# mttga/purejaxql

Hardware: NVIDIA H100
Metric: MinAtar-Breakout env steps/sec @4096 envs x128 seeds (higher is better)
Workload: dtype f32

## Files before the change

include/pqn_b200.h:

```cpp
#ifndef PQN_B200_H
#define PQN_B200_H

#include <stdint.h>

#ifdef __cplusplus
extern "C" {
#endif

#define PQN_OK 0
#define PQN_E_INVALID (-1)
#define PQN_E_CUDA (-2)
#define PQN_E_UNSUPPORTED (-3)

#define PQN_ENV_BREAKOUT 0
#define PQN_ENV_ASTERIX 1
#define PQN_ENV_SPACE_INVADERS 2
#define PQN_ENV_FREEWAY 3
#define PQN_ENV_SEAQUEST 4
#define PQN_ENV_CARTPOLE 16
#define PQN_ENV_ACROBOT 17
#define PQN_ENV_MEMORY_CHAIN 32

typedef struct pqn_env_info_t {
  int32_t state_words;
// ... 103 lines not shown
                 int32_t E, void* workspace, void* stream);
int pqn_rnn_loss_grad(const pqn_net_desc_t* desc_host, const float* params, const float* hs0, const float* obs,
                      const uint8_t* last_done, const int32_t* last_action, const int32_t* action, const float* reward,
                      const uint8_t* done, float* grads, float* loss_sum, float* qsa_sum, int32_t S, int32_t T, int32_t B,
                      float gamma, float lambda, void* workspace, void* stream);

int pqn_radam_clip_step(float* params, const float* grads, float* mu, float* nu, const float* sched,
                        int32_t* step_counter, float* gnorm_scratch , int32_t S, int64_t P,
                        float max_norm, float b1, float b2, float eps, void* stream);

int pqn_bn_stats_update(float* batch_stats, float* bn_sums, int32_t S, int32_t F, int64_t stats_seed_stride,
                        float count, float momentum, void* stream);

int pqn_set_tensor_core_path(int on);
int pqn_set_conv_mma_path(int on);

int pqn_tc_split_lo(const float* x, float* lo, int64_t n, void* stream);
int pqn_tc_gemm_test(const float* a, const float* a_lo, const float* b, const float* b_lo, float* d, int32_t S,
                     int32_t M, int32_t N, int32_t K, int a_mn, int b_mn, int split3, void* stream);

int pqn_tc_split16(const float* x, void* hi, void* lo, int64_t n, float scale, void* stream);
int pqn_tc_gemm16_test(const void* a_hi, const void* a_lo, const void* b_hi, const void* b_lo, float* d, int32_t S,
                       int32_t M, int32_t N, int32_t K, int a_mn, int b_mn, float out_scale, void* stream);
int pqn_tc_dgrad16_test(const void* a_hi, const void* a_lo, const void* b_hi, const void* b_lo, const float* mask,
                        const uint32_t* relu_bits, float* d, int32_t S, int32_t M, int32_t N, int32_t K, int epi,
                        float out_scale, void* stream);

#ifdef __cplusplus
}
#endif
// ... 2 lines not shown
```

purejaxql_b200/_lib.py:

```python
from __future__ import annotations

import ctypes
import os
from ctypes import POINTER, Structure, c_char_p, c_double, c_float, c_int, c_int32, c_int64, c_longlong, c_void_p

HERE = os.path.dirname(os.path.abspath(__file__))
LIB_PATH = os.path.join(HERE, "libpqn_b200.so")


class EnvInfo(Structure):
    _fields_ = [("state_words", c_int32), ("obs_dim", c_int32), ("obs_shape", c_int32 * 3),
                ("num_actions", c_int32), ("max_steps", c_int32), ("binary_obs", c_int32),
                ("packed_obs_words", c_int32)]


class EnvParams(Structure):
    _fields_ = [("max_steps", c_int32), ("memory_length", c_int32)]


class NetDesc(Structure):
    _fields_ = [("kind", c_int32), ("in_c", c_int32), ("hidden", c_int32), ("layers", c_int32),
                ("num_actions", c_int32), ("norm_type", c_int32), ("norm_input", c_int32)]


# ... 47 lines not shown
    "pqn_qnet_forward": (c_int, [POINTER(NetDesc), c_void_p, c_void_p, c_void_p, c_void_p, c_int64, c_void_p, c_int32,
                                 c_int64, c_void_p, c_void_p]),
    "pqn_qnet_loss_grad": (c_int, [POINTER(NetDesc), c_void_p, c_void_p, c_void_p, c_void_p, c_int64, c_void_p,
                                   c_void_p, c_int64, c_void_p, c_void_p, c_void_p, c_void_p, c_int32, c_int64,
                                   c_void_p, c_void_p]),
    "pqn_rnn_step": (c_int, [POINTER(NetDesc), c_void_p, c_void_p, c_void_p, c_int64, c_void_p, c_void_p, c_void_p,
                             c_int32, c_int32, c_void_p, c_void_p]),
    "pqn_rnn_loss_grad": (c_int, [POINTER(NetDesc), c_void_p, c_void_p, c_void_p, c_void_p, c_void_p, c_void_p, c_void_p,
                                  c_void_p, c_void_p, c_void_p, c_void_p, c_int32, c_int32, c_int32, c_float, c_float,
                                  c_void_p, c_void_p]),
    "pqn_radam_clip_step": (c_int, [c_void_p, c_void_p, c_void_p, c_void_p, c_void_p, c_void_p, c_void_p, c_int32,
                                    c_int64, c_float, c_float, c_float, c_float, c_void_p]),
    "pqn_bn_stats_update": (c_int, [c_void_p, c_void_p, c_int32, c_int32, c_int64, c_float, c_float, c_void_p]),
    "pqn_set_tensor_core_path": (c_int, [c_int]),
    "pqn_set_conv_mma_path": (c_int, [c_int]),
    "pqn_tc_split_lo": (c_int, [c_void_p, c_void_p, c_int64, c_void_p]),
    "pqn_tc_split16": (c_int, [c_void_p, c_void_p, c_void_p, c_int64, c_float, c_void_p]),
    "pqn_tc_gemm_test": (c_int, [c_void_p, c_void_p, c_void_p, c_void_p, c_void_p, c_int32, c_int32, c_int32,
                                 c_int32, c_int, c_int, c_int, c_void_p]),
    "pqn_tc_gemm16_test": (c_int, [c_void_p, c_void_p, c_void_p, c_void_p, c_void_p, c_int32, c_int32, c_int32,
                                   c_int32, c_int, c_int, c_float, c_void_p]),
    "pqn_tc_dgrad16_test": (c_int, [c_void_p, c_void_p, c_void_p, c_void_p, c_void_p, c_void_p, c_void_p, c_int32,
                                    c_int32, c_int32, c_int32, c_int, c_float, c_void_p]),
}

EXPORTS = tuple(_SIGS)
_lib = None


def lib():
# ... 52 lines not shown
```

purejaxql_b200/csrc/pqn_net.cu:

```cuda
#include <cuda_runtime.h>
#include <stdint.h>

#include "../../include/pqn_b200.h"
#include "api_common.h"
#include "tc_common.cuh"

namespace pqn {

constexpr int GT = 256;
constexpr int BK = 16;
constexpr float LN_EPS = 1e-6f;
constexpr int CONV_O = 16;
constexpr int CONV_PIX = 64;
constexpr int HID_CNN = 128;
constexpr int FLAT_CNN = CONV_PIX * CONV_O;

static int g_use_tc = 2;
static int g_conv_mma = 1;

static inline int64_t align4(int64_t x) { return (x + 3) & ~(int64_t)3; }

static int make_layout(const pqn_net_desc_t* d, pqn_net_layout_t* L) {
  int64_t off = 0;
  auto take = [&](int64_t n) { int64_t o = off; off += align4(n); return o; };
// ... 1003 lines not shown
    for (int h = 0; h < 2; ++h) {
      bl[h] = wb_lo[(ks * 2 + h) * 32 + lane];
      bh[h] = wb_hi[(ks * 2 + h) * 32 + lane];
    }
#pragma unroll
    for (int h = 0; h < 2; ++h)
#pragma unroll
      for (int i = 0; i < 2; ++i) mma_tf32_16n8k8(z[i][h], a[i], __float_as_uint(bl[h].x), __float_as_uint(bl[h].y));
#pragma unroll
    for (int h = 0; h < 2; ++h)
#pragma unroll
      for (int i = 0; i < 2; ++i) mma_tf32_16n8k8(z[i][h], a[i], __float_as_uint(bh[h].x), __float_as_uint(bh[h].y));
  }
}

__device__ __forceinline__ void ln16_quad(const float (&z)[2][4], float& mean0, float& rstd0, float& mean1,
                                          float& rstd1) {
  float s0 = z[0][0] + z[0][1] + z[1][0] + z[1][1];
  float q0 = z[0][0] * z[0][0] + z[0][1] * z[0][1] + z[1][0] * z[1][0] + z[1][1] * z[1][1];
  float s1 = z[0][2] + z[0][3] + z[1][2] + z[1][3];
  float q1 = z[0][2] * z[0][2] + z[0][3] * z[0][3] + z[1][2] * z[1][2] + z[1][3] * z[1][3];
#pragma unroll
  for (int o = 1; o <= 2; o <<= 1) {
    s0 += __shfl_xor_sync(0xffffffffu, s0, o); q0 += __shfl_xor_sync(0xffffffffu, q0, o);
    s1 += __shfl_xor_sync(0xffffffffu, s1, o); q1 += __shfl_xor_sync(0xffffffffu, q1, o);
  }
  mean0 = s0 * (1.0f / CONV_O); mean1 = s1 * (1.0f / CONV_O);
  rstd0 = rsqrtf(fmaxf(q0 * (1.0f / CONV_O) - mean0 * mean0, 0.f) + LN_EPS);
  rstd1 = rsqrtf(fmaxf(q1 * (1.0f / CONV_O) - mean1 * mean1, 0.f) + LN_EPS);
}

constexpr int CONV_MMA_WARPS = 8;

template <int C, bool TRAIN, bool H16 = false>
__global__ void __launch_bounds__(CONV_MMA_WARPS * 32, 3)
    conv_fwd_mma_kernel(const uint32_t* __restrict__ obs, int64_t obs_rows_per_seed, const int32_t* __restrict__ gather,
                        const float* __restrict__ params, int64_t P, pqn_net_layout_t L, float* __restrict__ H1,
                        float* __restrict__ H1LO, float* __restrict__ XH1, float* __restrict__ RS1,
                        uint32_t* __restrict__ RB, float* __restrict__ bn_sums, int rows) {
  using Cfg = ConvCfg<C>;
  using M = ConvMma<C>;
  __shared__ float2 wb_hi[M::KS * 2 * 32], wb_lo[M::KS * 2 * 32];
  __shared__ float cb[CONV_O], sc[CONV_O], bi[CONV_O];
  __shared__ uint32_t so[CONV_MMA_WARPS][Cfg::SW];
// ... 120 lines not shown
  }
}

__device__ __forceinline__ void mma_f16_16n8k16(float (&d)[4], const uint32_t (&a)[4], uint32_t b0, uint32_t b1) {
  asm volatile(
      "mma.sync.aligned.m16n8k16.row.col.f32.f16.f16.f32 {%0,%1,%2,%3}, {%4,%5,%6,%7}, {%8,%9}, {%0,%1,%2,%3};"
      : "+f"(d[0]), "+f"(d[1]), "+f"(d[2]), "+f"(d[3])
      : "r"(a[0]), "r"(a[1]), "r"(a[2]), "r"(a[3]), "r"(b0), "r"(b1));
}

template <int C>
struct Conv16 {
  static constexpr int TAPS = 9 * C;
  static constexpr int KS = (TAPS + 15) / 16;
  static constexpr int ROW = 2 * KS < 8 ? 8 : 2 * KS;
};

__host__ __device__ constexpr int conv16_channel(int h, int n) { return 4 * (n >> 1) + 2 * h + (n & 1); }

__host__ __device__ constexpr int conv16_tap(int s, int kk) {
  return 16 * s + (kk < 8 ? 0 : 8) + ((kk & 1) ? 4 : 0) + ((kk & 7) >> 1);
}

template <int C>
__device__ __forceinline__ void conv16_load_weights(const float* __restrict__ prm, const pqn_net_layout_t& L, uint4* wb,
                                                    float* cb, float* sc, float* bi) {
  using M = Conv16<C>;
  const float inv255 = 1.0f / 255.0f;
  for (int i = threadIdx.x; i < M::KS * 2 * 32; i += blockDim.x) {
    const int ln = i & 31, h = (i >> 5) & 1, s = i >> 6;
    const int gg = ln >> 2, tt = ln & 3;
    const int o = conv16_channel(h, gg);
    const float scale = __uint_as_float((uint32_t)(127 + 15 - (1 << tt)) << 23);
    float v[4];
#pragma unroll
    for (int q = 0; q < 4; ++q) {
      const int tap = conv16_tap(s, 2 * tt + (q & 1) + (q >> 1) * 8);
      v[q] = tap < M::TAPS ? __ldg(prm + L.conv_w + tap * CONV_O + o) * inv255 * scale : 0.f;
      v[q] = fminf(fmaxf(v[q], -65000.f), 65000.f);
    }
    const __half2 h0 = __floats2half2_rn(v[0], v[1]), h1 = __floats2half2_rn(v[2], v[3]);
    const float2 f0 = __half22float2(h0), f1 = __half22float2(h1);
    const __half2 l0 = __floats2half2_rn(v[0] - f0.x, v[1] - f0.y), l1 = __floats2half2_rn(v[2] - f1.x, v[3] - f1.y);
    wb[i] = make_uint4(*reinterpret_cast<const uint32_t*>(&h0), *reinterpret_cast<const uint32_t*>(&h1),
                       *reinterpret_cast<const uint32_t*>(&l0), *reinterpret_cast<const uint32_t*>(&l1));
  }
  if (threadIdx.x < CONV_O) {
    cb[threadIdx.x] = __ldg(prm + L.conv_b + threadIdx.x);
    sc[threadIdx.x] = __ldg(prm + L.ln0_scale + threadIdx.x);
    bi[threadIdx.x] = __ldg(prm + L.ln0_bias + threadIdx.x);
  }
}

template <int C>
__device__ __forceinline__ void build_patch16(const uint32_t* __restrict__ so, int pix, uint32_t* __restrict__ out) {
  constexpr int W = PatchCfg<C>::WORDS;
  uint32_t w[W];
  patch_bits<C>(so, pix, w);
#pragma unroll
  for (int b = 0; b < 2 * Conv16<C>::KS; ++b) {
    const int o = 8 * b;
    uint32_t v = (o >> 5) < W ? w[(o >> 5) < W ? (o >> 5) : 0] : 0u;
    const int sh = o & 31;
    const uint32_t lo = sh >= 10 ? v >> (sh - 10) : v << (10 - sh);
    const uint32_t hi = sh + 4 <= 26 ? v << (26 - sh - 4) : v >> (sh + 4 - 26);
// ... 26 lines not shown
      z[i][h][0] = z[i][h][2] = cb[4 * t + 2 * h];
      z[i][h][1] = z[i][h][3] = cb[4 * t + 2 * h + 1];
    }
  const uint32_t* r00 = xp + (32 * mbp + g) * M::ROW;
#pragma unroll
  for (int s = 0; s < M::KS; ++s) {
    uint32_t a[2][4];
#pragma unroll
    for (int i = 0; i < 2; ++i) {
      const uint2 w0 = *reinterpret_cast<const uint2*>(r00 + (16 * i) * M::ROW + 2 * s);
      const uint2 w1 = *reinterpret_cast<const uint2*>(r00 + (16 * i + 8) * M::ROW + 2 * s);
      a[i][0] = w0.x & mask; a[i][1] = w1.x & mask; a[i][2] = w0.y & mask; a[i][3] = w1.y & mask;
    }
    uint4 b[2];
#pragma unroll
    for (int h = 0; h < 2; ++h) b[h] = wb[(s * 2 + h) * 32 + lane];
#pragma unroll
    for (int h = 0; h < 2; ++h)
#pragma unroll
      for (int i = 0; i < 2; ++i) mma_f16_16n8k16(z[i][h], a[i], b[h].z, b[h].w);
#pragma unroll
    for (int h = 0; h < 2; ++h)
#pragma unroll
      for (int i = 0; i < 2; ++i) mma_f16_16n8k16(z[i][h], a[i], b[h].x, b[h].y);
  }
}

__device__ __forceinline__ uint32_t cvt_f16x2_satfinite(float lo, float hi) {
  uint32_t r;
  asm("cvt.rn.satfinite.f16x2.f32 %0, %1, %2;" : "=r"(r) : "f"(hi), "f"(lo));
  return r;
}

constexpr int CONV16_WARPS = 4;
constexpr int CONV16_CTAS_PER_SM = 5;

template <int C, bool TRAIN, bool H16>
__global__ void __launch_bounds__(CONV16_WARPS * 32, CONV16_CTAS_PER_SM)
    conv_fwd_mma16_kernel(const uint32_t* __restrict__ obs, int64_t obs_rows_per_seed, const int32_t* __restrict__ gather,
                          const float* __restrict__ params, int64_t P, pqn_net_layout_t L, float* __restrict__ H1,
                          float* __restrict__ H1LO, float* __restrict__ XH1, float* __restrict__ RS1,
                          uint32_t* __restrict__ RB, float* __restrict__ bn_sums, int rows) {
  using Cfg = ConvCfg<C>;
  using M = Conv16<C>;
  __shared__ __align__(16) uint4 wb[M::KS * 2 * 32];
  __shared__ float cb[CONV_O], sc[CONV_O], bi[CONV_O];
  __shared__ uint32_t so[CONV16_WARPS][Cfg::SW];
  __shared__ __align__(16) uint32_t sxp[CONV16_WARPS][CONV_PIX * M::ROW];
  __shared__ float s_cnt[C];
  const int tid = threadIdx.x, warp = tid >> 5, lane = tid & 31;
  const int g = lane >> 2, t = lane & 3;
  const int seed = blockIdx.y;
  conv16_load_weights<C>(params + (int64_t)seed * P, L, wb, cb, sc, bi);
  if (TRAIN && tid < C) s_cnt[tid] = 0.f;
  __syncthreads();
  int cnt[C];
  uint32_t cmask[C];
#pragma unroll
  for (int c = 0; c < C; ++c) {
    cnt[c] = 0;
// ... 31 lines not shown
    src_next = fetch_index(row + 2 * row_stride);
    store_patch16<C>(my_so, lane, sxp[warp] + lane * M::ROW);
    store_patch16<C>(my_so, lane + 32, sxp[warp] + (lane + 32) * M::ROW);
    __syncwarp();
    const int64_t grow = (int64_t)seed * rows + row;
    float* __restrict__ hrow = H16 ? nullptr : H1 + grow * FLAT_CNN;
    __half* __restrict__ hrow16 = H16 ? reinterpret_cast<__half*>(H1) + grow * FLAT_CNN : nullptr;
    __half* __restrict__ lrow16 = H16 ? reinterpret_cast<__half*>(H1LO) + grow * FLAT_CNN : nullptr;
    float* __restrict__ xrow = (TRAIN && XH1) ? XH1 + grow * FLAT_CNN : nullptr;
    float* __restrict__ rrow = (TRAIN && RS1) ? RS1 + grow * CONV_PIX : nullptr;
    uint16_t* __restrict__ brow = (TRAIN && RB) ? reinterpret_cast<uint16_t*>(RB + grow * (FLAT_CNN / 32)) : nullptr;
    float keep_rs0 = 0.f, keep_rs1 = 0.f;
    uint32_t keep_rb = 0u;
#pragma unroll 1
    for (int mbp = 0; mbp < 2; ++mbp) {
      float z2[2][2][4];
      conv16_block2<C>(sxp[warp], wb, cb, mbp, lane, z2);
#pragma unroll
      for (int mi = 0; mi < 2; ++mi) {
        const int mb = 2 * mbp + mi;
        float (&z)[2][4] = z2[mi];
        float mean0, rstd0, mean1, rstd1;
        ln16_quad(z, mean0, rstd0, mean1, rstd1);
        const float nm0 = -mean0 * rstd0, nm1 = -mean1 * rstd1;
        uint32_t rb0 = 0u, rb1 = 0u;
        const int p0 = 16 * mb + g, p1 = p0 + 8, o4 = 4 * t;
        float x0[4], x1[4], v0[4], v1[4];
#pragma unroll
        for (int h = 0; h < 2; ++h) {
#pragma unroll
          for (int c = 0; c < 2; ++c) {
            const int o = o4 + 2 * h + c;
            x0[2 * h + c] = fmaf(z[h][c], rstd0, nm0);
            x1[2 * h + c] = fmaf(z[h][2 + c], rstd1, nm1);
            v0[2 * h + c] = fmaxf(fmaf(x0[2 * h + c], sc[o], bi[o]), 0.f);
            v1[2 * h + c] = fmaxf(fmaf(x1[2 * h + c], sc[o], bi[o]), 0.f);
          }
        }
        if (H16) {
          uint32_t hw0[2], hw1[2], lw0[2], lw1[2];
#pragma unroll
          for (int h = 0; h < 2; ++h) {
            hw0[h] = cvt_f16x2_satfinite(v0[2 * h], v0[2 * h + 1]);
            hw1[h] = cvt_f16x2_satfinite(v1[2 * h], v1[2 * h + 1]);
            const float2 f0 = __half22float2(*reinterpret_cast<const __half2*>(&hw0[h]));
            const float2 f1 = __half22float2(*reinterpret_cast<const __half2*>(&hw1[h]));
            const __half2 l0 = __floats2half2_rn((v0[2 * h] - f0.x) * tc::TC_LO_SCALE, (v0[2 * h + 1] - f0.y) * tc::TC_LO_SCALE);
            const __half2 l1 = __floats2half2_rn((v1[2 * h] - f1.x) * tc::TC_LO_SCALE, (v1[2 * h + 1] - f1.y) * tc::TC_LO_SCALE);
            lw0[h] = *reinterpret_cast<const uint32_t*>(&l0); lw1[h] = *reinterpret_cast<const uint32_t*>(&l1);
          }
          *reinterpret_cast<uint2*>(hrow16 + p0 * CONV_O + o4) = make_uint2(hw0[0], hw0[1]);
          *reinterpret_cast<uint2*>(lrow16 + p0 * CONV_O + o4) = make_uint2(lw0[0], lw0[1]);
// ... 274 lines not shown
  }
  float* __restrict__ o = part + ((int64_t)seed * gridDim.x + blockIdx.x) * (M::TAPS * CONV_O + 3 * CONV_O);
  for (int i = tid; i < M::TAPS * CONV_O; i += blockDim.x) o[i] = s_w[i] * (1.0f / 255.0f);
  if (tid < 3 * CONV_O) o[M::TAPS * CONV_O + tid] = s_red[tid];
}

template <int C>
struct ConvBwd16 {
  static constexpr int MT = ConvMma<C>::MT;
  static constexpr int NG = 4 * MT;
  static constexpr int NGP = (NG % 8 == 4) ? NG : NG + 4;
  static constexpr int DY = 0;
  static constexpr int XH = DY + FLAT_CNN;
  static constexpr int RS = XH + FLAT_CNN;
  static constexpr int DZT = RS + CONV_PIX;
  static constexpr int PW = DZT + 2 * CONV_O * 32;
  static constexpr int WARP_FLOATS = (PW + 32 * NGP + 3) / 4 * 4;
  static constexpr int WARPS = (C == 4) ? 8 : 6;
  static constexpr int BYTES = (WARPS * WARP_FLOATS + 4 * CONV_O) * 4;
};

__device__ __forceinline__ int cswz16(int p, int col) {
  return ((p ^ ((p >> 2) & 1)) << 4) + (col ^ (((p >> 1) & 1) << 3));
}
__device__ __forceinline__ int dzt_word(int ch, int ks, int pos) {
  const int c7 = ch & 7;
  return (ch << 5) + ((ks ^ ((c7 + (c7 >> 2)) & 3)) << 3) + pos;
}

template <int C>
__global__ void __launch_bounds__(ConvBwd16<C>::WARPS * 32, 2)
    conv_bwd_mma16_kernel(const uint32_t* __restrict__ obs, int64_t obs_rows_per_seed, const int32_t* __restrict__ gather,
                          const float* __restrict__ params, int64_t P, pqn_net_layout_t L, const float* __restrict__ DY1,
                          const float* __restrict__ XH1, const float* __restrict__ RS1, float* __restrict__ part,
                          int rows, float gs) {
  using Cfg = ConvCfg<C>;
  using M = ConvMma<C>;
  using SM = ConvBwd16<C>;
  constexpr int PWD = PatchCfg<C>::WORDS;
  extern __shared__ __align__(16) float smem_bwd[];
  const int tid = threadIdx.x, warp = tid >> 5, lane = tid & 31;
  const int g = lane >> 2, t = lane & 3;
  const int seed = blockIdx.y;
  float* my = smem_bwd + warp * SM::WARP_FLOATS;
  float* my_dy = my + SM::DY;
  float* my_xh = my + SM::XH;
  float* my_rs = my + SM::RS;
  uint32_t* my_dzt = reinterpret_cast<uint32_t*>(my + SM::DZT);
  uint32_t* my_so = reinterpret_cast<uint32_t*>(my + SM::DZT);
  uint32_t* my_pw = reinterpret_cast<uint32_t*>(my + SM::PW);
  float* sc = smem_bwd + SM::WARPS * SM::WARP_FLOATS;
  float* s_red = sc + CONV_O;
  float* s_w = smem_bwd;
  static_assert(Cfg::SW <= 2 * CONV_O * 32, "obs staging aliases the dz planes");
  static_assert(M::MT * 16 * CONV_O <= SM::WARP_FLOATS * SM::WARPS, "dW reduction buffer aliases the warp slices");
  static_assert(Cfg::PW <= 32, "one packed observation word per lane");
  if (tid < CONV_O) sc[tid] = __ldg(params + (int64_t)seed * P + L.ln0_scale + tid);
  if (tid < 3 * CONV_O) s_red[tid] = 0.f;
  __syncthreads();
  float a_dsc[4] = {0.f, 0.f, 0.f, 0.f}, a_dbi[4] = {0.f, 0.f, 0.f, 0.f}, a_dcb[4] = {0.f, 0.f, 0.f, 0.f};
  float wrun[M::MT][2][4];
#pragma unroll
  for (int mt = 0; mt < M::MT; ++mt)
#pragma unroll
    for (int h = 0; h < 2; ++h)
#pragma unroll
      for (int j = 0; j < 4; ++j) wrun[mt][h][j] = 0.f;
  const uint32_t amask = (1u << (10 + (g & 3))) | (1u << (26 + (g & 3)));
  const int pos_g = g < 4 ? 2 * g : 2 * (g - 4) + 1;

  const int row_stride = gridDim.x * SM::WARPS;
  auto fetch_index = [&](int r) -> int {
    const int rc = r < rows ? r : rows - 1;
    return gather ? __ldg(gather + (int64_t)seed * rows + rc) : rc;
  };
  auto fetch_obs = [&](int src) -> uint32_t {
    return __ldg(obs + ((int64_t)seed * obs_rows_per_seed + src) * Cfg::PW + (lane < Cfg::PW ? lane : 0));
  };
  auto fetch_rows = [&](int r) {
    if (r < rows) {
      const int64_t gr = (int64_t)seed * rows + r;
      const float* dsrc = DY1 + gr * FLAT_CNN;
      const float* xsrc = XH1 + gr * FLAT_CNN;
#pragma unroll
      for (int i = 0; i < FLAT_CNN / 4 / 32; ++i) {
        const int q = i * 32 + lane, prow = q >> 2;
        const int dst = cswz16(prow, (q & 3) * 4);
        cp_async16(my_dy + dst, dsrc + q * 4);
        cp_async16(my_xh + dst, xsrc + q * 4);
      }
      if (lane < CONV_PIX / 4) cp_async16(my_rs + lane * 4, RS1 + gr * CONV_PIX + lane * 4);
    }
    cp_async_commit();
  };
  int row = blockIdx.x * SM::WARPS + warp;
  uint32_t pre = fetch_obs(fetch_index(row));
  int src_next = fetch_index(row + row_stride);
  fetch_rows(row);
  for (; row < rows; row += row_stride) {
    __syncwarp();
    if (lane < Cfg::PW) my_so[lane] = pre;
    if (lane == 0) my_so[Cfg::PW] = 0u;
    __syncwarp();
    pre = fetch_obs(src_next);
    src_next = fetch_index(row + 2 * row_stride);
    {
      uint32_t w0[PWD], w1[PWD];
      patch_bits<C>(my_so, 2 * lane, w0);
      patch_bits<C>(my_so, 2 * lane + 1, w1);
      uint32_t pw[SM::NGP];
#pragma unroll
      for (int k = 0; k < SM::NGP; ++k) pw[k] = 0u;
#pragma unroll
      for (int q = 0; q < SM::NG; ++q) {
        const int ql = q & 3, slot = (q & ~3) + (ql == 1 ? 2 : (ql == 2 ? 1 : ql));
        const int bit = 4 * q, wi = bit >> 5, sh = bit & 31;
        if (wi < PWD) {
          const uint32_t v0 = w0[wi < PWD ? wi : 0], v1 = w1[wi < PWD ? wi : 0];
          const uint32_t lo = sh >= 10 ? v0 >> (sh >= 10 ? sh - 10 : 0) : v0 << (sh < 10 ? 10 - sh : 0);
          const uint32_t hi = sh <= 26 ? v1 << (sh <= 26 ? 26 - sh : 0) : v1 >> (sh > 26 ? sh - 26 : 0);
          pw[slot] = __byte_perm(lo, hi, 0x7610);
        }
      }
      uint32_t* dstw = my_pw + lane * SM::NGP;
#pragma unroll
      for (int k = 0; k < SM::NGP / 4; ++k)
        *reinterpret_cast<uint4*>(dstw + 4 * k) = make_uint4(pw[4 * k], pw[4 * k + 1], pw[4 * k + 2], pw[4 * k + 3]);
    }
    cp_async_wait_all();
    __syncwarp();
#pragma unroll 1
    for (int mb = 0; mb < 4; ++mb) {
      const int p0 = 16 * mb + 2 * g, p1 = p0 + 1;
      float z[2][4];
      float2 dyv[2][2];
#pragma unroll
      for (int h = 0; h < 2; ++h) {
        dyv[h][0] = *reinterpret_cast<const float2*>(my_dy + cswz16(p0, 8 * h + 2 * t));
        dyv[h][1] = *reinterpret_cast<const float2*>(my_dy + cswz16(p1, 8 * h + 2 * t));
        const float2 a0 = *reinterpret_cast<const float2*>(my_xh + cswz16(p0, 8 * h + 2 * t));
        const float2 a1 = *reinterpret_cast<const float2*>(my_xh + cswz16(p1, 8 * h + 2 * t));
        z[h][0] = a0.x; z[h][1] = a0.y; z[h][2] = a1.x; z[h][3] = a1.y;
      }
// ... 68 lines not shown
        a[0] = wa.x & amask; a[1] = wa.y & amask; a[2] = wb.x & amask; a[3] = wb.y & amask;
        mma_f16_16n8k16(wacc[mt][0], a, blo[0].x, blo[0].y);
        mma_f16_16n8k16(wacc[mt][1], a, blo[1].x, blo[1].y);
        mma_f16_16n8k16(wacc[mt][0], a, bhi[0].x, bhi[0].y);
        mma_f16_16n8k16(wacc[mt][1], a, bhi[1].x, bhi[1].y);
      }
    }
#pragma unroll
    for (int mt = 0; mt < M::MT; ++mt)
#pragma unroll
      for (int h = 0; h < 2; ++h)
#pragma unroll
        for (int j = 0; j < 4; ++j) wrun[mt][h][j] += wacc[mt][h][j];
  }
  cp_async_wait_all();
  const float inv_gs = 1.0f / gs;
  const float unscale = __uint_as_float((uint32_t)(127 + 15 - (1 << (g & 3))) << 23) * inv_gs;
  __syncthreads();
  for (int w = 0; w < SM::WARPS; ++w) {
    if (warp == w) {
#pragma unroll
      for (int mt = 0; mt < M::MT; ++mt)
#pragma unroll
        for (int h = 0; h < 2; ++h)
#pragma unroll
          for (int j = 0; j < 4; ++j) {
            const int tap = 16 * mt + g + (j >= 2 ? 8 : 0);
            float* dst = &s_w[tap * CONV_O + 8 * h + 2 * t + (j & 1)];
            *dst = (w == 0 ? 0.f : *dst) + wrun[mt][h][j] * unscale;
          }
// ... 247 lines not shown
  if (cudaFuncSetAttribute(kfn, cudaFuncAttributeMaxDynamicSharedMemorySize, ConvBwdSmem<C>::BYTES) != cudaSuccess)
    return check_launch("conv_bwd_mma(cudaFuncSetAttribute)");
  kfn<<<grid, ConvBwdSmem<C>::WARPS * 32, ConvBwdSmem<C>::BYTES, st>>>(obs, orps, gather, params, P, L, dy1, xh1, rs1,
                                                                       part, rows);
  const int n = 9 * C * CONV_O + 3 * CONV_O;
  if (final_slices((int)grid.x) == 32)
    conv_bwd_final_kernel<32><<<dim3(cdiv(n, 8), grid.y), 256, 0, st>>>(part, (int)grid.x, 9 * C * CONV_O, grads, P, L);
  else
    conv_bwd_final_kernel<8><<<dim3(cdiv(n, 32), grid.y), 256, 0, st>>>(part, (int)grid.x, 9 * C * CONV_O, grads, P, L);
  return 0;
}

template <int C>
static int launch_conv_bwd_mma16(dim3 grid, cudaStream_t st, const uint32_t* obs, int64_t orps, const int32_t* gather,
                                 const float* params, int64_t P, const pqn_net_layout_t& L, const float* dy1,
                                 const float* xh1, const float* rs1, float* grads, float* part, int rows, float gs) {
  auto kfn = conv_bwd_mma16_kernel<C>;
  if (cudaFuncSetAttribute(kfn, cudaFuncAttributeMaxDynamicSharedMemorySize, ConvBwd16<C>::BYTES) != cudaSuccess)
    return check_launch("conv_bwd_mma16(cudaFuncSetAttribute)");
  kfn<<<grid, ConvBwd16<C>::WARPS * 32, ConvBwd16<C>::BYTES, st>>>(obs, orps, gather, params, P, L, dy1, xh1, rs1, part,
                                                                   rows, gs);
  const int n = 9 * C * CONV_O + 3 * CONV_O;
  if (final_slices((int)grid.x) == 32)
    conv_bwd_final_kernel<32><<<dim3(cdiv(n, 8), grid.y), 256, 0, st>>>(part, (int)grid.x, 9 * C * CONV_O, grads, P, L);
  else
    conv_bwd_final_kernel<8><<<dim3(cdiv(n, 32), grid.y), 256, 0, st>>>(part, (int)grid.x, 9 * C * CONV_O, grads, P, L);
  return 0;
}

static size_t row_bwd_smem(int N, int A, bool head) {
  return (size_t)(24 * N + (head ? A * N + 8 * A + 16 + 8 * A * N : 0)) * sizeof(float);
}
static int64_t row_bwd_part_floats(int N, int A) { return 3 * (int64_t)N + (int64_t)A * N + A + 2; }

template <int N, bool HEAD, typename... Args>
static int launch_row_bwd(dim3 grid, int A, cudaStream_t st, Args... args) {
// ... 329 lines not shown
  if ((rc = tc::make_tmap(&t[2], params + L.d0_w, HID_CNN, FLAT_CNN, S, HID_CNN, (uint64_t)P, 128))) return rc;
  if ((rc = tc::make_tmap(&t[3], w.w1_lo, HID_CNN, FLAT_CNN, S, HID_CNN, (uint64_t)FLAT_CNN * HID_CNN, 128))) return rc;
  tc::GemmShape gs = {};
  gs.S = S; gs.M = rows; gs.m_tiles = (rows + 127) / 128; gs.n_tiles = FLAT_CNN / 128; gs.k_blocks = HID_CNN / tc::TC_BK;
  gs.split3 = 1;
  tc::EpiParams ep = {};
  ep.out = w.h1; ep.mask = w.h1; ep.ld_out = FLAT_CNN; ep.out_seed_stride = (int64_t)rows * FLAT_CNN;
  ep.relu_bits = w.relu_bits; ep.rows = rows;
  return tc::launch_gemm(0, 0, have_bits ? tc::EPI_RELU_BITS : tc::EPI_RELU_MASK, t, gs, ep, st, K_TC_DGRAD);
}

#include "pqn_norm.cuh"
#include "pqn_rnn.cuh"

static inline bool modular_net(const pqn_net_desc_t* d) { return d->norm_type != PQN_NORM_LAYER || d->norm_input != 0; }

}

using namespace pqn;

extern "C" {

int64_t pqn_net_stats_floats(const pqn_net_desc_t* d) {
  if (check_desc(d, "pqn_net_stats_floats")) return -1;
  return nrm::stats_floats(d);
}

int pqn_rnn_step(const pqn_net_desc_t* d, const float* params, float* hs, const float* obs, int64_t obs_rows_per_seed,
                 const uint8_t* last_done, const int32_t* last_action, float* q, int32_t S, int32_t E, void* workspace,
                 void* stream) {
// ... 95 lines not shown
  return check_launch("pqn_rnn_loss_grad");
}

int pqn_set_conv_mma_path(int on) {
  if (on != 0 && on != 1 && on != 3) return set_error(PQN_E_UNSUPPORTED, "pqn_set_conv_mma_path: no conv path %d", on);
  g_conv_mma = on;
  return PQN_OK;
}

int pqn_set_tensor_core_path(int on) {
  if (on < 0 || on > 2) return set_error(PQN_E_UNSUPPORTED, "pqn_set_tensor_core_path: no tensor-core path %d", on);
  g_use_tc = on;
  return PQN_OK;
}

int pqn_net_layout(const pqn_net_desc_t* d, pqn_net_layout_t* out) {
  int rc = check_desc(d, "pqn_net_layout");
  if (rc) return rc;
  if (!out) return set_error(PQN_E_INVALID, "pqn_net_layout: out is NULL");
  make_layout(d, out);
  return PQN_OK;
}

int64_t pqn_net_workspace_bytes(const pqn_net_desc_t* d, int32_t S, int64_t rows) {
  if (check_desc(d, "pqn_net_workspace_bytes")) return -1;
  if (d->kind == PQN_NET_RNN) return rnn::carve_rnn(d, S, rows, nullptr, nullptr);
  if (modular_net(d)) return nrm::carve_norm(d, S, rows, nullptr, nullptr);
  return carve(d, S, rows, nullptr, nullptr);
}

// ... 96 lines not shown
    nrm::NormWs nw;
    nrm::carve_norm(d, S, rows, (char*)workspace, &nw);
    return nrm::norm_loss_grad(d, L, params, batch_stats, obs, gather, obs_rows_per_seed, action, target, tr_rows_per_seed,
                              grads, loss_sum, qsa_sum, bn_sums, S, R, nw, st);
  }

  if (d->kind == PQN_NET_MINATAR_CNN) {
    const uint32_t* ob = (const uint32_t*)obs;
    const bool use_tc = g_use_tc && A <= PQN_TC_MAX_A;
    const bool f16 = use_tc && g_use_tc == 2;
    const Planes16 pl = planes16(w, S, rows);
    const bool conv16 = f16 && g_conv_mma == 1;
    const float gscale = f16 ? grad_scale(rows) : 1.0f;
    launch_conv_fwd<true>(d->in_c, dim3(cdiv(rows, 4), S), st, ob, obs_rows_per_seed, gather, params, P, L,
                          conv16 ? (float*)pl.h1_hi : w.h1, conv16 ? (float*)pl.h1_lo : nullptr, bn_sums, R,
                          g_conv_mma ? w.cxhat : nullptr, g_conv_mma ? w.crstd : nullptr,
                          (g_conv_mma == 1 || g_conv_mma == 3) ? w.relu_bits : nullptr, conv16);
    if (f16) {
      if (!conv16) launch_split16_h1(w.h1, pl, (int64_t)S * rows * FLAT_CNN, st);
      launch_split16_w1(params, P, L.d0_w, pl, S, st);
      if ((rc = tc16_dense_fwd(tc::EPI_LN_TRAIN, params, P, L, w, pl, A, nullptr, S, R, st))) return rc;
    } else if (use_tc) {
      launch_split_w1(params, P, L.d0_w, w.w1_lo, S, st);
      if ((rc = tc_dense_fwd(tc::EPI_LN_TRAIN, params, P, L, w, A, nullptr, S, R, st))) return rc;
    } else {
      launch_dense<1>(128, dim3(cdiv(rows, 128), S), st, w.h1, rows * FLAT_CNN, FLAT_CNN, params, P, L.d0_w, L.d0_b,
                      L.ln1_scale, L.ln1_bias, 0, 0, A, w.h2, w.xhat2, w.rstd2, nullptr, R, FLAT_CNN);
    }
    const dim3 rbg(conv_mma_ctas(S, R, 4), S);
    if ((rc = run_row_bwd(128, true, rbg, A, st, w.h2, w.xhat2, w.rstd2, nullptr, w.dz2, (use_tc && !f16) ? w.dz2_lo : nullptr,
                          f16 ? pl.dz_hi : nullptr, f16 ? pl.dz_lo : nullptr, gscale, params, grads, P, L.ln1_scale,
// ... 7 lines not shown
      if ((rc = tc_dgrad(params, P, L, w, S, R, g_conv_mma == 1 || g_conv_mma == 3, st))) return rc;
    } else {
      const int splits = wgrad_splits(FLAT_CNN / 128, S, R);
      run_wgrad_ffma(w.h1, rows * FLAT_CNN, FLAT_CNN, w.dz2, rows * HID_CNN, HID_CNN, grads, P, L.d0_w, R, FLAT_CNN, S, splits, w.wg_part, st);
      { LaunchScope _ls(K_DGRAD, st); dgrad_kernel<<<dim3(cdiv(rows, 128), FLAT_CNN / 128, S), GT, 0, st>>>(w.dz2, rows * HID_CNN, HID_CNN, params, P,
                                                                            L.d0_w, w.h1, w.h1, rows * FLAT_CNN, R,
                                                                            FLAT_CNN); }
    }
    dim3 cg(conv_bwd_ctas(S, R), S);
    if (g_conv_mma) {
      const dim3 mg(conv_mma_ctas(S, R, 2), S);
      LaunchScope _ls(K_CONV_BWD, st);
      const float gs16 = grad_scale((int)rows) * (1.0f / 16.0f);
      if (g_conv_mma == 1) {
        switch (d->in_c) {
          case 4: rc = launch_conv_bwd_mma16<4>(mg, st, ob, obs_rows_per_seed, gather, params, P, L, w.h1, w.cxhat, w.crstd, grads, w.cb_part, R, gs16); break;
          case 6: rc = launch_conv_bwd_mma16<6>(mg, st, ob, obs_rows_per_seed, gather, params, P, L, w.h1, w.cxhat, w.crstd, grads, w.cb_part, R, gs16); break;
          case 7: rc = launch_conv_bwd_mma16<7>(mg, st, ob, obs_rows_per_seed, gather, params, P, L, w.h1, w.cxhat, w.crstd, grads, w.cb_part, R, gs16); break;
          case 10: rc = launch_conv_bwd_mma16<10>(mg, st, ob, obs_rows_per_seed, gather, params, P, L, w.h1, w.cxhat, w.crstd, grads, w.cb_part, R, gs16); break;
        }
      } else
      switch (d->in_c) {
        case 4: rc = launch_conv_bwd_mma<4>(mg, st, ob, obs_rows_per_seed, gather, params, P, L, w.h1, w.cxhat, w.crstd, grads, w.cb_part, R); break;
        case 6: rc = launch_conv_bwd_mma<6>(mg, st, ob, obs_rows_per_seed, gather, params, P, L, w.h1, w.cxhat, w.crstd, grads, w.cb_part, R); break;
        case 7: rc = launch_conv_bwd_mma<7>(mg, st, ob, obs_rows_per_seed, gather, params, P, L, w.h1, w.cxhat, w.crstd, grads, w.cb_part, R); break;
        case 10: rc = launch_conv_bwd_mma<10>(mg, st, ob, obs_rows_per_seed, gather, params, P, L, w.h1, w.cxhat, w.crstd, grads, w.cb_part, R); break;
      }
      if (rc) return rc;
    } else
    switch (d->in_c) {
      case 4: { LaunchScope _ls(K_CONV_BWD, st); conv_bwd_kernel<4><<<cg, 256, 0, st>>>(ob, obs_rows_per_seed, gather, params, P, L, w.h1, grads, R); } break;
      case 6: { LaunchScope _ls(K_CONV_BWD, st); conv_bwd_kernel<6><<<cg, 256, 0, st>>>(ob, obs_rows_per_seed, gather, params, P, L, w.h1, grads, R); } break;
      case 7: { LaunchScope _ls(K_CONV_BWD, st); conv_bwd_kernel<7><<<cg, 256, 0, st>>>(ob, obs_rows_per_seed, gather, params, P, L, w.h1, grads, R); } break;
      case 10: { LaunchScope _ls(K_CONV_BWD, st); conv_bwd_kernel<10><<<cg, 256, 0, st>>>(ob, obs_rows_per_seed, gather, params, P, L, w.h1, grads, R); } break;
// ... 56 lines not shown
```

Baseline: 33.46 million.

## Recompute conv LayerNorm xhat/rstd in f16 conv backward instead of storing them

The forward conv kernel no longer writes the normalized conv activations (xhat) and rstd to global memory in conv_mma mode 1. The backward MMA kernel instead reloads the conv weights into shared memory, rebuilds the input patches and recomputes xhat/rstd with the same f16 split MMA path. This trades a large global write plus a later read per row for extra tensor-core compute and more shared memory per CTA. Deterministic fma rounding is used so the recomputed values match the forward ones, and a test entry point compares the two. It also packs the last weight K-slice in half to save shared memory.

```diff
diff --git a/include/pqn_b200.h b/include/pqn_b200.h
--- a/include/pqn_b200.h
+++ b/include/pqn_b200.h
@@ -141,6 +141,9 @@
 
 int pqn_set_tensor_core_path(int on);
 int pqn_set_conv_mma_path(int on);
+int pqn_conv16_xhat_test(const pqn_net_desc_t* desc_host, const float* params, const void* obs, const int32_t* gather,
+                         int64_t obs_rows_per_seed, int32_t S, int64_t rows, float* fwd_xhat, float* fwd_rstd,
+                         float* rec_xhat, float* rec_rstd, void* workspace, void* stream);
 
 int pqn_tc_split_lo(const float* x, float* lo, int64_t n, void* stream);
 int pqn_tc_gemm_test(const float* a, const float* a_lo, const float* b, const float* b_lo, float* d, int32_t S,
diff --git a/purejaxql_b200/_lib.py b/purejaxql_b200/_lib.py
--- a/purejaxql_b200/_lib.py
+++ b/purejaxql_b200/_lib.py
@@ -85,6 +85,8 @@
     "pqn_bn_stats_update": (c_int, [c_void_p, c_void_p, c_int32, c_int32, c_int64, c_float, c_float, c_void_p]),
     "pqn_set_tensor_core_path": (c_int, [c_int]),
     "pqn_set_conv_mma_path": (c_int, [c_int]),
+    "pqn_conv16_xhat_test": (c_int, [POINTER(NetDesc), c_void_p, c_void_p, c_void_p, c_int64, c_int32, c_int64,
+                                     c_void_p, c_void_p, c_void_p, c_void_p, c_void_p, c_void_p]),
     "pqn_tc_split_lo": (c_int, [c_void_p, c_void_p, c_int64, c_void_p]),
     "pqn_tc_split16": (c_int, [c_void_p, c_void_p, c_void_p, c_int64, c_float, c_void_p]),
     "pqn_tc_gemm_test": (c_int, [c_void_p, c_void_p, c_void_p, c_void_p, c_void_p, c_int32, c_int32, c_int32,
diff --git a/purejaxql_b200/csrc/pqn_net.cu b/purejaxql_b200/csrc/pqn_net.cu
--- a/purejaxql_b200/csrc/pqn_net.cu
+++ b/purejaxql_b200/csrc/pqn_net.cu
@@ -1041,20 +1041,23 @@
   }
 }
 
+__device__ __forceinline__ float sumsq4(float a, float b, float c, float d) {
+  return __fmaf_rn(d, d, __fmaf_rn(c, c, __fmaf_rn(a, a, __fmul_rn(b, b))));
+}
 __device__ __forceinline__ void ln16_quad(const float (&z)[2][4], float& mean0, float& rstd0, float& mean1,
                                           float& rstd1) {
   float s0 = z[0][0] + z[0][1] + z[1][0] + z[1][1];
-  float q0 = z[0][0] * z[0][0] + z[0][1] * z[0][1] + z[1][0] * z[1][0] + z[1][1] * z[1][1];
+  float q0 = sumsq4(z[0][0], z[0][1], z[1][0], z[1][1]);
   float s1 = z[0][2] + z[0][3] + z[1][2] + z[1][3];
-  float q1 = z[0][2] * z[0][2] + z[0][3] * z[0][3] + z[1][2] * z[1][2] + z[1][3] * z[1][3];
+  float q1 = sumsq4(z[0][2], z[0][3], z[1][2], z[1][3]);
 #pragma unroll
   for (int o = 1; o <= 2; o <<= 1) {
     s0 += __shfl_xor_sync(0xffffffffu, s0, o); q0 += __shfl_xor_sync(0xffffffffu, q0, o);
     s1 += __shfl_xor_sync(0xffffffffu, s1, o); q1 += __shfl_xor_sync(0xffffffffu, q1, o);
   }
   mean0 = s0 * (1.0f / CONV_O); mean1 = s1 * (1.0f / CONV_O);
-  rstd0 = rsqrtf(fmaxf(q0 * (1.0f / CONV_O) - mean0 * mean0, 0.f) + LN_EPS);
-  rstd1 = rsqrtf(fmaxf(q1 * (1.0f / CONV_O) - mean1 * mean1, 0.f) + LN_EPS);
+  rstd0 = rsqrtf(fmaxf(__fmaf_rn(q0, 1.0f / CONV_O, -__fmul_rn(mean0, mean0)), 0.f) + LN_EPS);
+  rstd1 = rsqrtf(fmaxf(__fmaf_rn(q1, 1.0f / CONV_O, -__fmul_rn(mean1, mean1)), 0.f) + LN_EPS);
 }
 
 constexpr int CONV_MMA_WARPS = 8;
@@ -1205,6 +1208,8 @@
   static constexpr int TAPS = 9 * C;
   static constexpr int KS = (TAPS + 15) / 16;
   static constexpr int ROW = 2 * KS < 8 ? 8 : 2 * KS;
+  static constexpr bool LAST_B0_ONLY = 16 * (KS - 1) + 8 >= TAPS;
+  static constexpr int WB_BYTES = ((KS - 1) * 64 + (LAST_B0_ONLY ? 32 : 64)) * 16;
 };
 
 __host__ __device__ constexpr int conv16_channel(int h, int n) { return 4 * (n >> 1) + 2 * h + (n & 1); }
@@ -1233,13 +1238,17 @@
     const __half2 h0 = __floats2half2_rn(v[0], v[1]), h1 = __floats2half2_rn(v[2], v[3]);
     const float2 f0 = __half22float2(h0), f1 = __half22float2(h1);
     const __half2 l0 = __floats2half2_rn(v[0] - f0.x, v[1] - f0.y), l1 = __floats2half2_rn(v[2] - f1.x, v[3] - f1.y);
-    wb[i] = make_uint4(*reinterpret_cast<const uint32_t*>(&h0), *reinterpret_cast<const uint32_t*>(&h1),
-                       *reinterpret_cast<const uint32_t*>(&l0), *reinterpret_cast<const uint32_t*>(&l1));
+    if (M::LAST_B0_ONLY && s == M::KS - 1)
+      reinterpret_cast<uint2*>(wb + (M::KS - 1) * 64)[i & 63] =
+          make_uint2(*reinterpret_cast<const uint32_t*>(&h0), *reinterpret_cast<const uint32_t*>(&l0));
+    else
+      wb[i] = make_uint4(*reinterpret_cast<const uint32_t*>(&h0), *reinterpret_cast<const uint32_t*>(&h1),
+                         *reinterpret_cast<const uint32_t*>(&l0), *reinterpret_cast<const uint32_t*>(&l1));
   }
   if (threadIdx.x < CONV_O) {
     cb[threadIdx.x] = __ldg(prm + L.conv_b + threadIdx.x);
-    sc[threadIdx.x] = __ldg(prm + L.ln0_scale + threadIdx.x);
-    bi[threadIdx.x] = __ldg(prm + L.ln0_bias + threadIdx.x);
+    if (sc) sc[threadIdx.x] = __ldg(prm + L.ln0_scale + threadIdx.x);
+    if (bi) bi[threadIdx.x] = __ldg(prm + L.ln0_bias + threadIdx.x);
   }
 }
 
@@ -1296,7 +1305,14 @@
     }
     uint4 b[2];
 #pragma unroll
-    for (int h = 0; h < 2; ++h) b[h] = wb[(s * 2 + h) * 32 + lane];
+    for (int h = 0; h < 2; ++h) {
+      if (M::LAST_B0_ONLY && s == M::KS - 1) {
+        const uint2 v = reinterpret_cast<const uint2*>(wb + (M::KS - 1) * 64)[h * 32 + lane];
+        b[h] = make_uint4(v.x, 0u, v.y, 0u);
+      } else {
+        b[h] = wb[(s * 2 + h) * 32 + lane];
+      }
+    }
 #pragma unroll
     for (int h = 0; h < 2; ++h)
 #pragma unroll
@@ -1305,6 +1321,30 @@
     for (int h = 0; h < 2; ++h)
 #pragma unroll
       for (int i = 0; i < 2; ++i) mma_f16_16n8k16(z[i][h], a[i], b[h].x, b[h].y);
+  }
+}
+
+template <int C>
+__device__ __forceinline__ void conv16_xhat_block2(const uint32_t* __restrict__ xp, const uint4* __restrict__ wb,
+                                                   const float* __restrict__ cb, int mbp, int lane,
+                                                   float (&xh)[2][2][4], float (&rs)[2][2]) {
+  float z2[2][2][4];
+  conv16_block2<C>(xp, wb, cb, mbp, lane, z2);
+#pragma unroll
+  for (int mi = 0; mi < 2; ++mi) {
+    const float (&z)[2][4] = z2[mi];
+    float mean0, rstd0, mean1, rstd1;
+    ln16_quad(z, mean0, rstd0, mean1, rstd1);
+    const float nm0 = -__fmul_rn(mean0, rstd0), nm1 = -__fmul_rn(mean1, rstd1);
+#pragma unroll
+    for (int h = 0; h < 2; ++h)
+#pragma unroll
+      for (int c = 0; c < 2; ++c) {
+        xh[mi][0][2 * h + c] = __fmaf_rn(z[h][c], rstd0, nm0);
+        xh[mi][1][2 * h + c] = __fmaf_rn(z[h][2 + c], rstd1, nm1);
+      }
+    rs[mi][0] = rstd0;
+    rs[mi][1] = rstd1;
   }
 }
 
@@ -1325,7 +1365,7 @@
                           uint32_t* __restrict__ RB, float* __restrict__ bn_sums, int rows) {
   using Cfg = ConvCfg<C>;
   using M = Conv16<C>;
-  __shared__ __align__(16) uint4 wb[M::KS * 2 * 32];
+  __shared__ __align__(16) uint4 wb[M::WB_BYTES / 16];
   __shared__ float cb[CONV_O], sc[CONV_O], bi[CONV_O];
   __shared__ uint32_t so[CONV16_WARPS][Cfg::SW];
   __shared__ __align__(16) uint32_t sxp[CONV16_WARPS][CONV_PIX * M::ROW];
@@ -1387,28 +1427,20 @@
     uint32_t keep_rb = 0u;
 #pragma unroll 1
     for (int mbp = 0; mbp < 2; ++mbp) {
-      float z2[2][2][4];
-      conv16_block2<C>(sxp[warp], wb, cb, mbp, lane, z2);
+      float xh[2][2][4], rs[2][2];
+      conv16_xhat_block2<C>(sxp[warp], wb, cb, mbp, lane, xh, rs);
 #pragma unroll
       for (int mi = 0; mi < 2; ++mi) {
         const int mb = 2 * mbp + mi;
-        float (&z)[2][4] = z2[mi];
-        float mean0, rstd0, mean1, rstd1;
-        ln16_quad(z, mean0, rstd0, mean1, rstd1);
-        const float nm0 = -mean0 * rstd0, nm1 = -mean1 * rstd1;
+        const float rstd0 = rs[mi][0], rstd1 = rs[mi][1];
         uint32_t rb0 = 0u, rb1 = 0u;
         const int p0 = 16 * mb + g, p1 = p0 + 8, o4 = 4 * t;
-        float x0[4], x1[4], v0[4], v1[4];
-#pragma unroll
-        for (int h = 0; h < 2; ++h) {
-#pragma unroll
-          for (int c = 0; c < 2; ++c) {
-            const int o = o4 + 2 * h + c;
-            x0[2 * h + c] = fmaf(z[h][c], rstd0, nm0);
-            x1[2 * h + c] = fmaf(z[h][2 + c], rstd1, nm1);
-            v0[2 * h + c] = fmaxf(fmaf(x0[2 * h + c], sc[o], bi[o]), 0.f);
-            v1[2 * h + c] = fmaxf(fmaf(x1[2 * h + c], sc[o], bi[o]), 0.f);
-          }
+        const float (&x0)[4] = xh[mi][0], (&x1)[4] = xh[mi][1];
+        float v0[4], v1[4];
+#pragma unroll
+        for (int c = 0; c < 4; ++c) {
+          v0[c] = fmaxf(fmaf(x0[c], sc[o4 + c], bi[o4 + c]), 0.f);
+          v1[c] = fmaxf(fmaf(x1[c], sc[o4 + c], bi[o4 + c]), 0.f);
         }
         if (H16) {
           uint32_t hw0[2], hw1[2], lw0[2], lw1[2];
@@ -1713,10 +1745,14 @@
   static constexpr int XH = DY + FLAT_CNN;
   static constexpr int RS = XH + FLAT_CNN;
   static constexpr int DZT = RS + CONV_PIX;
+  static constexpr int XP = 64;
   static constexpr int PW = DZT + 2 * CONV_O * 32;
   static constexpr int WARP_FLOATS = (PW + 32 * NGP + 3) / 4 * 4;
   static constexpr int WARPS = (C == 4) ? 8 : 6;
-  static constexpr int BYTES = (WARPS * WARP_FLOATS + 4 * CONV_O) * 4;
+  static constexpr int BYTES = (WARPS * WARP_FLOATS + 5 * CONV_O) * 4 + Conv16<C>::WB_BYTES;
+  static_assert(ConvCfg<C>::SW <= XP && XP + CONV_PIX * Conv16<C>::ROW <= 2 * CONV_O * 32,
+                "patch rows fit in the dz planes behind the obs row");
+  static_assert(2 * (BYTES + 1024) <= 228 * 1024, "two CTAs per SM (1 KB per CTA is reserved)");
 };
 
 __device__ __forceinline__ int cswz16(int p, int col) {
@@ -1727,12 +1763,12 @@
   return (ch << 5) + ((ks ^ ((c7 + (c7 >> 2)) & 3)) << 3) + pos;
 }
 
-template <int C>
+template <int C, bool EXPORT = false>
 __global__ void __launch_bounds__(ConvBwd16<C>::WARPS * 32, 2)
     conv_bwd_mma16_kernel(const uint32_t* __restrict__ obs, int64_t obs_rows_per_seed, const int32_t* __restrict__ gather,
                           const float* __restrict__ params, int64_t P, pqn_net_layout_t L, const float* __restrict__ DY1,
-                          const float* __restrict__ XH1, const float* __restrict__ RS1, float* __restrict__ part,
-                          int rows, float gs) {
+                          float* __restrict__ part, int rows, float gs, float* __restrict__ XH_OUT,
+                          float* __restrict__ RS_OUT) {
   using Cfg = ConvCfg<C>;
   using M = ConvMma<C>;
   using SM = ConvBwd16<C>;
@@ -1747,14 +1783,16 @@
   float* my_rs = my + SM::RS;
   uint32_t* my_dzt = reinterpret_cast<uint32_t*>(my + SM::DZT);
   uint32_t* my_so = reinterpret_cast<uint32_t*>(my + SM::DZT);
+  uint32_t* my_xp = my_so + SM::XP;
   uint32_t* my_pw = reinterpret_cast<uint32_t*>(my + SM::PW);
   float* sc = smem_bwd + SM::WARPS * SM::WARP_FLOATS;
   float* s_red = sc + CONV_O;
+  float* cb = s_red + 3 * CONV_O;
+  const uint4* wb = reinterpret_cast<const uint4*>(cb + CONV_O);
   float* s_w = smem_bwd;
-  static_assert(Cfg::SW <= 2 * CONV_O * 32, "obs staging aliases the dz planes");
   static_assert(M::MT * 16 * CONV_O <= SM::WARP_FLOATS * SM::WARPS, "dW reduction buffer aliases the warp slices");
   static_assert(Cfg::PW <= 32, "one packed observation word per lane");
-  if (tid < CONV_O) sc[tid] = __ldg(params + (int64_t)seed * P + L.ln0_scale + tid);
+  conv16_load_weights<C>(params + (int64_t)seed * P, L, reinterpret_cast<uint4*>(cb + CONV_O), cb, sc, nullptr);
   if (tid < 3 * CONV_O) s_red[tid] = 0.f;
   __syncthreads();
   float a_dsc[4] = {0.f, 0.f, 0.f, 0.f}, a_dbi[4] = {0.f, 0.f, 0.f, 0.f}, a_dcb[4] = {0.f, 0.f, 0.f, 0.f};
@@ -1777,18 +1815,13 @@
     return __ldg(obs + ((int64_t)seed * obs_rows_per_seed + src) * Cfg::PW + (lane < Cfg::PW ? lane : 0));
   };
   auto fetch_rows = [&](int r) {
-    if (r < rows) {
-      const int64_t gr = (int64_t)seed * rows + r;
-      const float* dsrc = DY1 + gr * FLAT_CNN;
-      const float* xsrc = XH1 + gr * FLAT_CNN;
+    if (!EXPORT && r < rows) {
+      const float* dsrc = DY1 + ((int64_t)seed * rows + r) * FLAT_CNN;
 #pragma unroll
       for (int i = 0; i < FLAT_CNN / 4 / 32; ++i) {
         const int q = i * 32 + lane, prow = q >> 2;
-        const int dst = cswz16(prow, (q & 3) * 4);
-        cp_async16(my_dy + dst, dsrc + q * 4);
-        cp_async16(my_xh + dst, xsrc + q * 4);
-      }
-      if (lane < CONV_PIX / 4) cp_async16(my_rs + lane * 4, RS1 + gr * CONV_PIX + lane * 4);
+        cp_async16(my_dy + cswz16(prow, (q & 3) * 4), dsrc + q * 4);
+      }
     }
     cp_async_commit();
   };
@@ -1803,6 +1836,8 @@
     __syncwarp();
     pre = fetch_obs(src_next);
     src_next = fetch_index(row + 2 * row_stride);
+    store_patch16<C>(my_so, lane, my_xp + lane * Conv16<C>::ROW);
+    store_patch16<C>(my_so, lane + 32, my_xp + (lane + 32) * Conv16<C>::ROW);
     {
       uint32_t w0[PWD], w1[PWD];
       patch_bits<C>(my_so, 2 * lane, w0);
@@ -1826,6 +1861,28 @@
       for (int k = 0; k < SM::NGP / 4; ++k)
         *reinterpret_cast<uint4*>(dstw + 4 * k) = make_uint4(pw[4 * k], pw[4 * k + 1], pw[4 * k + 2], pw[4 * k + 3]);
     }
+    __syncwarp();
+#pragma unroll
+    for (int mbp = 0; mbp < 2; ++mbp) {
+      float xh[2][2][4], rs[2][2];
+      conv16_xhat_block2<C>(my_xp, wb, cb, mbp, lane, xh, rs);
+#pragma unroll
+      for (int mi = 0; mi < 2; ++mi)
+#pragma unroll
+        for (int r = 0; r < 2; ++r) {
+          const int p = 32 * mbp + 16 * mi + 8 * r + g;
+          *reinterpret_cast<float4*>(my_xh + cswz16(p, 4 * t)) =
+              make_float4(xh[mi][r][0], xh[mi][r][1], xh[mi][r][2], xh[mi][r][3]);
+          if (t == 0) my_rs[p] = rs[mi][r];
+        }
+    }
+    if (EXPORT) {
+      __syncwarp();
+      const int64_t gr = (int64_t)seed * rows + row;
+      for (int i = lane; i < FLAT_CNN; i += 32) XH_OUT[gr * FLAT_CNN + i] = my_xh[cswz16(i >> 4, i & 15)];
+      for (int i = lane; i < CONV_PIX; i += 32) RS_OUT[gr * CONV_PIX + i] = my_rs[i];
+      continue;
+    }
     cp_async_wait_all();
     __syncwarp();
 #pragma unroll 1
@@ -1924,6 +1981,7 @@
         for (int j = 0; j < 4; ++j) wrun[mt][h][j] += wacc[mt][h][j];
   }
   cp_async_wait_all();
+  if (EXPORT) return;
   const float inv_gs = 1.0f / gs;
   const float unscale = __uint_as_float((uint32_t)(127 + 15 - (1 << (g & 3))) << 23) * inv_gs;
   __syncthreads();
@@ -2201,12 +2259,12 @@
 template <int C>
 static int launch_conv_bwd_mma16(dim3 grid, cudaStream_t st, const uint32_t* obs, int64_t orps, const int32_t* gather,
                                  const float* params, int64_t P, const pqn_net_layout_t& L, const float* dy1,
-                                 const float* xh1, const float* rs1, float* grads, float* part, int rows, float gs) {
+                                 float* grads, float* part, int rows, float gs) {
   auto kfn = conv_bwd_mma16_kernel<C>;
   if (cudaFuncSetAttribute(kfn, cudaFuncAttributeMaxDynamicSharedMemorySize, ConvBwd16<C>::BYTES) != cudaSuccess)
     return check_launch("conv_bwd_mma16(cudaFuncSetAttribute)");
-  kfn<<<grid, ConvBwd16<C>::WARPS * 32, ConvBwd16<C>::BYTES, st>>>(obs, orps, gather, params, P, L, dy1, xh1, rs1, part,
-                                                                   rows, gs);
+  kfn<<<grid, ConvBwd16<C>::WARPS * 32, ConvBwd16<C>::BYTES, st>>>(obs, orps, gather, params, P, L, dy1, part, rows, gs,
+                                                                   nullptr, nullptr);
   const int n = 9 * C * CONV_O + 3 * CONV_O;
   if (final_slices((int)grid.x) == 32)
     conv_bwd_final_kernel<32><<<dim3(cdiv(n, 8), grid.y), 256, 0, st>>>(part, (int)grid.x, 9 * C * CONV_O, grads, P, L);
@@ -2566,6 +2624,21 @@
 #include "pqn_rnn.cuh"
 
 static inline bool modular_net(const pqn_net_desc_t* d) { return d->norm_type != PQN_NORM_LAYER || d->norm_input != 0; }
+
+template <int C>
+static int conv16_xhat_test(const uint32_t* obs, int64_t orps, const int32_t* gather, const float* params, int64_t P,
+                            const pqn_net_layout_t& L, const Planes16& pl, int S, int rows, float* fx, float* fr,
+                            float* rx, float* rr, cudaStream_t st) {
+  const dim3 fg(conv_mma_ctas(S, rows, CONV16_CTAS_PER_SM), S);
+  conv_fwd_mma16_kernel<C, true, true><<<fg, CONV16_WARPS * 32, 0, st>>>(
+      obs, orps, gather, params, P, L, (float*)pl.h1_hi, (float*)pl.h1_lo, fx, fr, nullptr, nullptr, rows);
+  auto kfn = conv_bwd_mma16_kernel<C, true>;
+  if (cudaFuncSetAttribute(kfn, cudaFuncAttributeMaxDynamicSharedMemorySize, ConvBwd16<C>::BYTES) != cudaSuccess)
+    return check_launch("pqn_conv16_xhat_test(cudaFuncSetAttribute)");
+  kfn<<<dim3(conv_mma_ctas(S, rows, 2), S), ConvBwd16<C>::WARPS * 32, ConvBwd16<C>::BYTES, st>>>(
+      obs, orps, gather, params, P, L, nullptr, nullptr, rows, 1.0f, rx, rr);
+  return check_launch("pqn_conv16_xhat_test");
+}
 
 }
 
@@ -2691,6 +2764,33 @@
   return PQN_OK;
 }
 
+int pqn_conv16_xhat_test(const pqn_net_desc_t* d, const float* params, const void* obs, const int32_t* gather,
+                         int64_t obs_rows_per_seed, int32_t S, int64_t rows, float* fwd_xhat, float* fwd_rstd,
+                         float* rec_xhat, float* rec_rstd, void* workspace, void* stream) {
+  int rc = check_desc(d, "pqn_conv16_xhat_test");
+  if (rc) return rc;
+  if (d->kind != PQN_NET_MINATAR_CNN || modular_net(d) || !params || !obs || !fwd_xhat || !fwd_rstd || !rec_xhat ||
+      !rec_rstd || !workspace || S <= 0 || S > 65535 || rows <= 0 || rows > 0x7fffffff)
+    return set_error(PQN_E_INVALID, "pqn_conv16_xhat_test: bad argument");
+  pqn_net_layout_t L;
+  make_layout(d, &L);
+  Workspace w;
+  carve(d, S, rows, (char*)workspace, &w);
+  const Planes16 pl = planes16(w, S, rows);
+  const uint32_t* ob = (const uint32_t*)obs;
+  const cudaStream_t st = (cudaStream_t)stream;
+#define PQN_XT(CC) conv16_xhat_test<CC>(ob, obs_rows_per_seed, gather, params, L.total, L, pl, S, (int)rows, fwd_xhat, \
+                                        fwd_rstd, rec_xhat, rec_rstd, st)
+  switch (d->in_c) {
+    case 4: return PQN_XT(4);
+    case 6: return PQN_XT(6);
+    case 7: return PQN_XT(7);
+    case 10: return PQN_XT(10);
+    default: return set_error(PQN_E_UNSUPPORTED, "pqn_conv16_xhat_test: %d input channels", d->in_c);
+  }
+#undef PQN_XT
+}
+
 int pqn_net_layout(const pqn_net_desc_t* d, pqn_net_layout_t* out) {
   int rc = check_desc(d, "pqn_net_layout");
   if (rc) return rc;
@@ -2817,7 +2917,7 @@
     const float gscale = f16 ? grad_scale(rows) : 1.0f;
     launch_conv_fwd<true>(d->in_c, dim3(cdiv(rows, 4), S), st, ob, obs_rows_per_seed, gather, params, P, L,
                           conv16 ? (float*)pl.h1_hi : w.h1, conv16 ? (float*)pl.h1_lo : nullptr, bn_sums, R,
-                          g_conv_mma ? w.cxhat : nullptr, g_conv_mma ? w.crstd : nullptr,
+                          g_conv_mma == 3 ? w.cxhat : nullptr, g_conv_mma == 3 ? w.crstd : nullptr,
                           (g_conv_mma == 1 || g_conv_mma == 3) ? w.relu_bits : nullptr, conv16);
     if (f16) {
       if (!conv16) launch_split16_h1(w.h1, pl, (int64_t)S * rows * FLAT_CNN, st);
@@ -2855,10 +2955,10 @@
       const float gs16 = grad_scale((int)rows) * (1.0f / 16.0f);
       if (g_conv_mma == 1) {
         switch (d->in_c) {
-          case 4: rc = launch_conv_bwd_mma16<4>(mg, st, ob, obs_rows_per_seed, gather, params, P, L, w.h1, w.cxhat, w.crstd, grads, w.cb_part, R, gs16); break;
-          case 6: rc = launch_conv_bwd_mma16<6>(mg, st, ob, obs_rows_per_seed, gather, params, P, L, w.h1, w.cxhat, w.crstd, grads, w.cb_part, R, gs16); break;
-          case 7: rc = launch_conv_bwd_mma16<7>(mg, st, ob, obs_rows_per_seed, gather, params, P, L, w.h1, w.cxhat, w.crstd, grads, w.cb_part, R, gs16); break;
-          case 10: rc = launch_conv_bwd_mma16<10>(mg, st, ob, obs_rows_per_seed, gather, params, P, L, w.h1, w.cxhat, w.crstd, grads, w.cb_part, R, gs16); break;
+          case 4: rc = launch_conv_bwd_mma16<4>(mg, st, ob, obs_rows_per_seed, gather, params, P, L, w.h1, grads, w.cb_part, R, gs16); break;
+          case 6: rc = launch_conv_bwd_mma16<6>(mg, st, ob, obs_rows_per_seed, gather, params, P, L, w.h1, grads, w.cb_part, R, gs16); break;
+          case 7: rc = launch_conv_bwd_mma16<7>(mg, st, ob, obs_rows_per_seed, gather, params, P, L, w.h1, grads, w.cb_part, R, gs16); break;
+          case 10: rc = launch_conv_bwd_mma16<10>(mg, st, ob, obs_rows_per_seed, gather, params, P, L, w.h1, grads, w.cb_part, R, gs16); break;
         }
       } else
       switch (d->in_c) {
```

New measurement: 35.45 million, median of 6. +5.9%, better.
